# jgsimard/big-dreamer

Hardware: AMD Instinct MI355X
Metric: latent transitions/sec (RSSM + imagination) at batch=50 chunk=50 H=15 (higher is better)
Workload: dtype f32

## Files before the change

### big_dreamer_amd/csrc/bd_device.h

```cpp
#pragma once
#include <hip/hip_runtime.h>
#include <stdint.h>

#include "../../include/bigdreamer_hip.h"

namespace bd {

typedef float floatx4 __attribute__((ext_vector_type(4)));

#ifndef BD_WAVES
#define BD_WAVES 4
#endif
constexpr int kWaves = BD_WAVES;
constexpr int kThreads = kWaves * 64;
constexpr int kFragFloats = 256;

__device__ __forceinline__ floatx4 mfma16(float a, float b, floatx4 c) {
    return __builtin_amdgcn_mfma_f32_16x16x4f32(a, b, c, 0, 0, 0);
}

__host__ __device__ __forceinline__ int cdiv(int a, int b) { return (a + b - 1) / b; }

__device__ __forceinline__ int bd_tid() {
    int t = threadIdx.x;
// ... 313 lines not shown
                return f;
            },
            [&](const LinFrag<RT, NI>& f) {
                if constexpr (kSplit) {
                    if constexpr (TR) {
                        acc[0][0] = mfma16(f.b[0][0], f.a[0][0], acc[0][0]);
                        acc2 = mfma16(f.b[0][1], f.a[0][1], acc2);
                        acc[0][0] = mfma16(f.b[0][2], f.a[0][2], acc[0][0]);
                        acc2 = mfma16(f.b[0][3], f.a[0][3], acc2);
                    } else {
                        acc[0][0] = mfma16(f.a[0][0], f.b[0][0], acc[0][0]);
                        acc2 = mfma16(f.a[0][1], f.b[0][1], acc2);
                        acc[0][0] = mfma16(f.a[0][2], f.b[0][2], acc[0][0]);
                        acc2 = mfma16(f.a[0][3], f.b[0][3], acc2);
                    }
                } else {
#pragma unroll
                    for (int j = 0; j < 4; ++j)
#pragma unroll
                        for (int i = 0; i < NI; ++i)
#pragma unroll
                            for (int rt = 0; rt < RT; ++rt)
                                acc[i][rt] = TR ? mfma16(f.b[i][j], f.a[rt][j], acc[i][rt]) : mfma16(f.a[rt][j], f.b[i][j], acc[i][rt]);
                }
            });
    }
    if constexpr (kSplit) acc[0][0] += acc2;
}

template <int NSEG, int RT, int NI, int D, bool TR = false, class Pre, class Epi>
__device__ __forceinline__ void linear_blocks(const Seg (&seg)[NSEG], const float* __restrict__ bias, int N, int nb0,
                                              Pre&& pre, Epi&& epi, int sb = -1) {
    const int lane = bd_tid() & 63;
    BD_DSTAMP(sb, 0);
    decltype(pre(0, 0)) pf[NI][RT];
#pragma unroll
    for (int i = 0; i < NI; ++i)
#pragma unroll
        for (int rt = 0; rt < RT; ++rt) pf[i][rt] = pre(rt, nb0 + i * kWaves);
    floatx4 acc[NI][RT];
#pragma unroll
    for (int i = 0; i < NI; ++i) {
        floatx4 b4;
        if constexpr (TR) {
            b4 = tall_bias(bias, N, nb0 + i * kWaves, lane);
        } else {
            const int col = (nb0 + i * kWaves) * 16 + (lane & 15);
            const float b = (bias != nullptr && col < N) ? bias[col] : 0.f;
            b4 = floatx4{b, b, b, b};
        }
#pragma unroll
        for (int rt = 0; rt < RT; ++rt) acc[i][rt] = b4;
    }
    BD_DSTAMP(sb, 1);
    linear_sweep<NSEG, RT, NI, D, TR>(seg, nb0, acc);
    BD_DSTAMP(sb, 2);
#pragma unroll
    for (int i = 0; i < NI; ++i)
#pragma unroll
        for (int rt = 0; rt < RT; ++rt) epi(rt, nb0 + i * kWaves, acc[i][rt], pf[i][rt]);
    BD_DSTAMP(sb, 3);
}

constexpr int kSplitPairs = 2;
constexpr int kHeadMaxN = 64;
constexpr int kHeadPlainFloats = 2 * 16 * kHeadMaxN;
constexpr int kSplitPartialFloats = kWaves * kSplitPairs * 2 * kFragFloats;
constexpr int kSplitScratchFloats = kSplitPartialFloats + kHeadPlainFloats;

template <int RT, int NSEG, bool TR = false, class Pre, class Epi>
__device__ __forceinline__ void tile_linear_splitk(const Seg (&seg)[NSEG], const float* __restrict__ bias, int N,
                                                   float* __restrict__ scratch, Pre&& pre, Epi&& epi) {
    const int lane = bd_tid() & 63, wave = bd_wave(bd_tid());
    const int Nb = (N + 15) >> 4;
    const int P = Nb * RT;
    const int my_nb = wave / RT, my_rt = wave - my_nb * RT;
    decltype(pre(0, 0)) pf{};
    floatx4 my_bias = floatx4{0.f, 0.f, 0.f, 0.f};
    if (wave < P) {
        pf = pre(my_rt, my_nb);
        if constexpr (TR) {
            my_bias = tall_bias(bias, N, my_nb, lane);
        } else {
            const int col = my_nb * 16 + (lane & 15);
            const float b = (bias != nullptr && col < N) ? bias[col] : 0.f;
            my_bias = floatx4{b, b, b, b};
        }
    }
    floatx4 acc[kSplitPairs];
#pragma unroll
    for (int p = 0; p < kSplitPairs; ++p) acc[p] = floatx4{0.f, 0.f, 0.f, 0.f};
    constexpr int KW = 2;
#pragma unroll
    for (int s = 0; s < NSEG; ++s) {
        const int Kb = seg[s].Kb;
        const floatx4* __restrict__ X4 = reinterpret_cast<const floatx4*>(seg[s].X) + lane;
        const floatx4* __restrict__ W4 = reinterpret_cast<const floatx4*>(seg[s].W) + lane;
        for (int kb0 = wave; kb0 < Kb; kb0 += kWaves * KW) {
            floatx4 xa[KW][kSplitPairs], wb[KW][kSplitPairs];
#pragma unroll
            for (int i = 0; i < KW; ++i) {
                const int kb = kb0 + i * kWaves;
#pragma unroll
                for (int p = 0; p < kSplitPairs; ++p) {
                    if (kb < Kb && p < P) {
                        const int nb = p / RT, rt = p % RT;
                        xa[i][p] = X4[(rt * Kb + kb) * 64];
                        wb[i][p] = W4[((size_t)nb * Kb + kb) * 64];
                    }
                }
            }
#pragma unroll
            for (int i = 0; i < KW; ++i) {
                const int kb = kb0 + i * kWaves;
#pragma unroll
                for (int p = 0; p < kSplitPairs; ++p) {
                    if (kb < Kb && p < P) {
#pragma unroll
                        for (int j = 0; j < 4; ++j)
                            acc[p] = TR ? mfma16(wb[i][p][j], xa[i][p][j], acc[p]) : mfma16(xa[i][p][j], wb[i][p][j], acc[p]);
                    }
                }
            }
        }
    }
    floatx4* __restrict__ S4 = reinterpret_cast<floatx4*>(scratch);
#pragma unroll
    for (int p = 0; p < kSplitPairs; ++p)
        if (p < P) S4[(wave * kSplitPairs + p) * 64 + lane] = acc[p];
    lds_barrier();
    if (wave < P) {
        floatx4 r = my_bias;
        for (int w = 0; w < kWaves; ++w) r += S4[(w * kSplitPairs + wave) * 64 + lane];
        epi(my_rt, my_nb, r, pf);
    }
}

template <int RT, int NSEG, bool TR = false, class Pre, class Epi>
__device__ __forceinline__ void tile_linear_pre(const Seg (&seg)[NSEG], const float* __restrict__ bias, int N, Pre&& pre,
                                                Epi&& epi, float* __restrict__ scratch = nullptr, int sb = -1) {
    const int wave = bd_wave(bd_tid());
    const int Nb = (N + 15) >> 4;
    if (scratch != nullptr && Nb * RT <= kSplitPairs) {
        tile_linear_splitk<RT, NSEG, TR>(seg, bias, N, scratch, pre, epi);
        return;
    }
#ifndef BD_PIPE_D
#define BD_PIPE_D 2
#endif
    constexpr int D = BD_PIPE_D;
    for (int nb0 = wave; nb0 < Nb; nb0 += 2 * kWaves) {
        if (nb0 + kWaves < Nb) linear_blocks<NSEG, RT, 2, D, TR>(seg, bias, N, nb0, pre, epi, sb);
        else linear_blocks<NSEG, RT, 1, D, TR>(seg, bias, N, nb0, pre, epi, sb);
    }
}

template <int RT, int NSEG, class Epi>
__device__ __forceinline__ void tile_linear_g(const Seg (&seg)[NSEG], const float* __restrict__ bias, int N, Epi&& epi,
                                              float* __restrict__ scratch = nullptr, int sb = -1) {
    tile_linear_pre<RT, NSEG>(seg, bias, N, NoPre{}, [&](int rt, int nb, floatx4 acc, NoPreVal) { epi(rt, nb, acc); },
                              scratch, sb);
}

template <int RT, class Epi>
__device__ __forceinline__ void tile_linear(const float* __restrict__ X, int Kb, const float* __restrict__ Wp,
                                            const float* __restrict__ bias, int N, Epi&& epi,
                                            float* __restrict__ scratch = nullptr) {
    const Seg seg[1] = {{X, Wp, Kb}};
    tile_linear_g<RT, 1>(seg, bias, N, epi, scratch);
}

template <int NSEG, class Epi>
__device__ __forceinline__ void tile_linear_seg(const Seg (&seg)[NSEG], const float* __restrict__ bias, int N,
                                                Epi&& epi, float* __restrict__ scratch = nullptr, int sb = -1) {
    tile_linear_g<1, NSEG>(seg, bias, N, [&](int, int nb, floatx4 acc) { epi(nb, acc); }, scratch, sb);
}
template <int NSEG, class Epi>
__device__ __forceinline__ void tile_linear_seg_tr(const Seg (&seg)[NSEG], const float* __restrict__ bias, int N, Epi&& epi,
                                                   int sb = -1) {
    tile_linear_pre<1, NSEG, true>(seg, bias, N, NoPre{}, [&](int, int nb, floatx4 acc, NoPreVal) { epi(nb, acc); }, nullptr, sb);
}

constexpr int kTallMaxPer = 3;

template <int RT>
struct TallAcc {
    floatx4 main[kTallMaxPer][RT];
    floatx4 left;
};

__host__ __device__ __forceinline__ bool tall_shape_ok(int N, int RT) {
    const int Nb = (N + 15) >> 4, per = Nb / kWaves;
    return per <= kTallMaxPer && (Nb - per * kWaves) * RT <= kWaves;
}

__device__ __forceinline__ bool tall_left_pair(int Nb, int RT, int wave, int& rt, int& nb) {
    const int per = Nb / kWaves, nleft = (Nb - per * kWaves) * RT;
    if (wave >= nleft) return false;
    const int lb = wave / RT;
    rt = wave - lb * RT;
    nb = per * kWaves + lb;
    return true;
}

template <int RT, int NSEG>
__device__ __forceinline__ void tall_sweep(const Seg (&seg)[NSEG], const float* __restrict__ bias, int N, TallAcc<RT>& t) {
    const int lane = bd_tid() & 63, wave = bd_wave(bd_tid());
    const int Nb = (N + 15) >> 4, per = Nb / kWaves;
#pragma unroll
    for (int i = 0; i < kTallMaxPer; ++i) {
        const floatx4 b = i < per ? tall_bias(bias, N, wave + i * kWaves, lane) : floatx4{0.f, 0.f, 0.f, 0.f};
#pragma unroll
        for (int rt = 0; rt < RT; ++rt) t.main[i][rt] = b;
    }
    if (per == 3) linear_sweep<NSEG, RT, 3, 1, true>(seg, wave, t.main);
    else if (per == 2) linear_sweep<NSEG, RT, 2, 1, true>(seg, wave, t.main);
    else if (per == 1) linear_sweep<NSEG, RT, 1, 2, true>(seg, wave, t.main);
    int lrt = 0, lnb = 0;
    if (tall_left_pair(Nb, RT, wave, lrt, lnb)) {
        floatx4 one[1][1] = {{tall_bias(bias, N, lnb, lane)}};
        Seg s1[NSEG];
#pragma unroll
        for (int s = 0; s < NSEG; ++s) s1[s] = Seg{seg[s].X + (size_t)lrt * seg[s].Kb * kFragFloats, seg[s].W, seg[s].Kb};
        linear_sweep<NSEG, 1, 1, 2, true>(s1, lnb, one);
        t.left = one[0][0];
    }
}

template <int RT, class F>
__device__ __forceinline__ void tall_foreach(int N, const TallAcc<RT>& t, F&& f) {
    const int wave = bd_wave(bd_tid());
    const int Nb = (N + 15) >> 4, per = Nb / kWaves;
#pragma unroll
    for (int i = 0; i < kTallMaxPer; ++i)
        if (i < per) {
#pragma unroll
            for (int rt = 0; rt < RT; ++rt) f(rt, wave + i * kWaves, t.main[i][rt]);
        }
    int lrt = 0, lnb = 0;
    if (tall_left_pair(Nb, RT, wave, lrt, lnb)) f(lrt, lnb, t.left);
}

template <int RT, class G>
__device__ __forceinline__ void tall_fill(int N, TallAcc<RT>& t, G&& g) {
    const int wave = bd_wave(bd_tid());
    const int Nb = (N + 15) >> 4, per = Nb / kWaves;
#pragma unroll
    for (int i = 0; i < kTallMaxPer; ++i)
        if (i < per) {
#pragma unroll
            for (int rt = 0; rt < RT; ++rt) t.main[i][rt] = g(rt, wave + i * kWaves);
        }
    int lrt = 0, lnb = 0;
    if (tall_left_pair(Nb, RT, wave, lrt, lnb)) t.left = g(lrt, lnb);
}

template <int RT, class F>
__device__ __forceinline__ void tall_foreach2(int N, const TallAcc<RT>& t, const TallAcc<RT>& u, F&& f) {
    const int wave = bd_wave(bd_tid());
    const int Nb = (N + 15) >> 4, per = Nb / kWaves;
#pragma unroll
    for (int i = 0; i < kTallMaxPer; ++i)
        if (i < per) {
#pragma unroll
            for (int rt = 0; rt < RT; ++rt) f(rt, wave + i * kWaves, t.main[i][rt], u.main[i][rt]);
        }
    int lrt = 0, lnb = 0;
    if (tall_left_pair(Nb, RT, wave, lrt, lnb)) f(lrt, lnb, t.left, u.left);
}

struct Seg2 {
    const float* X;
    const float* W0;
    const float* W1;
    int Kb;
};

struct DualFrag {
    floatx4 a, p, q;
};

template <int NSEG, class Pre, class Epi>
__device__ __forceinline__ void tile_linear_dual_pre(const Seg2 (&seg)[NSEG], const float* __restrict__ bias0,
                                                     const float* __restrict__ bias1, int N, Pre&& pre, Epi&& epi,
                                                     float* __restrict__ scratch = nullptr, int sb = -1) {
    const int lane = bd_tid() & 63, wave = bd_wave(bd_tid());
    const int Nb = (N + 15) >> 4;
    if (scratch != nullptr && Nb <= kSplitPairs) {
        BD_DSTAMP(sb, 0);
        decltype(pre(0)) pf{};
        float mb0 = 0.f, mb1 = 0.f;
        if (wave < Nb) {
            pf = pre(wave);
            const int col = wave * 16 + (lane & 15);
            mb0 = (bias0 != nullptr && col < N) ? bias0[col] : 0.f;
            mb1 = (bias1 != nullptr && col < N) ? bias1[col] : 0.f;
        }
        floatx4 a0[kSplitPairs], a1[kSplitPairs];
#pragma unroll
        for (int p = 0; p < kSplitPairs; ++p) a0[p] = a1[p] = floatx4{0.f, 0.f, 0.f, 0.f};
        constexpr int KW = 2;
#pragma unroll
        for (int s = 0; s < NSEG; ++s) {
            const int Kb = seg[s].Kb;
            const floatx4* __restrict__ X4 = reinterpret_cast<const floatx4*>(seg[s].X) + lane;
            const floatx4* __restrict__ W0 = reinterpret_cast<const floatx4*>(seg[s].W0) + lane;
// ... 359 lines not shown
```

### big_dreamer_amd/csrc/bd_scan.h

```cpp
#pragma once
#include "bd_device.h"

namespace bd {

struct EntConst {
    float mean, sd, inv_var, inv_sd, base0;
};
__device__ __forceinline__ EntConst entropy_const(float mean, float sd) {
    constexpr float kLogSqrt2Pi = 0.91893853320467274f, kLn2 = 0.69314718055994531f;
    return EntConst{mean, sd, 1.f / (sd * sd), 1.f / sd, -logf(sd) - kLogSqrt2Pi - 2.f * kLn2};
}
__device__ __forceinline__ void entropy_sample(const EntConst& c, float e, float& lp, float& dm, float& ds) {
    constexpr float kClamp = 0.99999994f;
    const float u = c.mean + c.sd * e;
    const float y = tanhf(u);
    const float yc = fminf(fmaxf(y, -kClamp), kClamp);
    const float a = 1.f + yc, b = 1.f - yc;
    const float xh = 0.5f * logf(a / b);
    const float diff = xh - c.mean;
    const float t = -2.f * xh;
    const float ex = expf(t);
    const float sp = t > 20.f ? t : log1pf(ex);
    const float sg = t > 20.f ? 1.f : ex / (1.f + ex);
    lp = c.base0 - 0.5f * diff * diff * c.inv_var + 2.f * (xh + sp);
    const float gx = -diff * c.inv_var + 2.f - 4.f * sg;
    const bool pass = (y >= -kClamp) && (y <= kClamp);
    const float J = pass ? (1.f - y * y) / (a * b) : 0.f;
    dm = diff * c.inv_var + gx * J;
    ds = diff * diff * c.inv_var * c.inv_sd - c.inv_sd + gx * J * e;
}


struct HiddenEpi {
    float* dst;
    float* save;
    size_t tn;
    int width, rows, row0, lane;
    __device__ __forceinline__ void operator()(int nb, floatx4 acc) const {
        const int c = lane & 15, q = lane >> 4;
        float* __restrict__ p = dst + acc_frag_off(nb, lane, 0);
        if (row0 + 16 <= rows && nb * 16 + 16 <= width) {
            float v[4];
#pragma unroll
            for (int r = 0; r < 4; ++r) v[r] = elu(acc[r]);
#pragma unroll
            for (int r = 0; r < 4; ++r) p[4 * r] = v[r];
            if (save) {
                float* __restrict__ s = save + tn * width + ((unsigned)(row0 + 4 * q) * (unsigned)width + (unsigned)(nb * 16 + c));
#pragma unroll
                for (int r = 0; r < 4; ++r) st_save(s + (unsigned)r * (unsigned)width, v[r]);
            }
            return;
        }
        const int col = nb * 16 + c;
#pragma unroll
        for (int r = 0; r < 4; ++r) {
            const int grow = row0 + 4 * q + r;
            const bool ok = grow < rows && col < width;
            const float v = ok ? elu(acc[r]) : 0.f;
            p[4 * r] = v;
            if (ok && save) save[(tn + grow) * width + col] = v;
        }
    }
};

struct HiddenEpiTR {
    float* dst;
    float* save;
    size_t tn;
    int width, rows, row0, lane;
    __device__ __forceinline__ void operator()(int nb, floatx4 acc) const {
        const int row = lane & 15, col0 = nb * 16 + 4 * (lane >> 4);
        const bool rok = row0 + row < rows;
        floatx4 v;
#pragma unroll
        for (int r = 0; r < 4; ++r) v[r] = (rok && col0 + r < width) ? elu(acc[r]) : 0.f;
        reinterpret_cast<floatx4*>(dst)[nb * 64 + lane] = v;
        if (save && rok && col0 < width) {
            float* __restrict__ s = save + (tn + row0 + row) * width + col0;
            if (col0 + 4 <= width) {
                __builtin_memcpy(s, &v, 16);
            } else {
#pragma unroll
                for (int r = 0; r < 4; ++r)
                    if (col0 + r < width) s[r] = v[r];
            }
        }
    }
};

struct DpreEpi {
    float* dst;
    float* out;
    size_t tn;
    int width, rows, row0, lane;
    __device__ __forceinline__ void operator()(int, int nb, floatx4 acc, const Pre4& p) const {
        const int c = lane & 15, q = lane >> 4;
        if (row0 + 16 <= rows && nb * 16 + 16 <= width) {
            float v[4];
#pragma unroll
            for (int r = 0; r < 4; ++r) v[r] = acc[r] * elu_grad_from_out(p.v[r]);
            if (out) {
                float* __restrict__ s = out + tn * width + ((unsigned)(row0 + 4 * q) * (unsigned)width + (unsigned)(nb * 16 + c));
#pragma unroll
                for (int r = 0; r < 4; ++r) s[(unsigned)r * (unsigned)width] = v[r];
            }
            if (dst) {
                float* __restrict__ w = dst + acc_frag_off(nb, lane, 0);
#pragma unroll
                for (int r = 0; r < 4; ++r) w[4 * r] = v[r];
            }
            return;
        }
        const int col = nb * 16 + c;
#pragma unroll
        for (int r = 0; r < 4; ++r) {
            const int grow = row0 + 4 * q + r;
            float v = 0.f;
            if (grow < rows && col < width) {
                v = acc[r] * elu_grad_from_out(p.v[r]);
                if (out) out[(tn + grow) * width + col] = v;
            }
            if (dst) dst[acc_frag_off(nb, lane, r)] = v;
        }
    }
};
struct DprePre {
    const float* saved;
    size_t tn;
    int width, rows, row0, lane;
    __device__ __forceinline__ Pre4 operator()(int, int nb) const {
        Pre4 p;
        const int c = lane & 15, q = lane >> 4;
        if (row0 + 16 <= rows && nb * 16 + 16 <= width) {
            const float* __restrict__ s = saved + tn * width + ((unsigned)(row0 + 4 * q) * (unsigned)width + (unsigned)(nb * 16 + c));
#pragma unroll
            for (int r = 0; r < 4; ++r) p.v[r] = s[(unsigned)r * (unsigned)width];
            return p;
        }
        const int col = nb * 16 + c;
#pragma unroll
        for (int r = 0; r < 4; ++r) {
            const int grow = row0 + 4 * q + r;
            p.v[r] = (grow < rows && col < width) ? saved[(tn + grow) * width + col] : 1.f;
        }
        return p;
    }
};

struct PreAct {
    float act[4], th[4], sg[4], dm[4], ds[4], eps[4];
};

}
```

### big_dreamer_amd/csrc/imagine.hip

```cpp
#include "bd_device.h"
#include "bd_host.h"
#include "bd_scan.h"
#include "bd_rng.h"
#include "bd_discrete.h"

namespace bd {

constexpr int kMaxA = 64;

#ifdef BD_STAMPS
__device__ unsigned long long g_stamps[64];
#define BD_STAMP(slot)                                                                      \
    do {                                                                                    \
        if (blockIdx.x == BD_STAMP_WG && threadIdx.x == 0 && t == 3) g_stamps[slot] = __builtin_amdgcn_s_memtime(); \
    } while (0)
#ifndef BD_STAMP_WG
#define BD_STAMP_WG 0
#endif
#else
#define BD_STAMP(slot)
#endif

struct ImgDims {
    int Kb_h, Kb_s, Kb_a, Kb_hd;
// ... 200 lines not shown
                const bool ok = grow < a.N && col < a.Be;
                h_nxt[off] = ok ? hn : 0.f;
                if (ok) {
                    a.feat[(tn + grow) * F + col] = hn;
                    if (a.sv_gates) {
                        float* g = a.sv_gates + (tn + grow) * 4 * a.Be + col;
                        g[0] = rr; g[a.Be] = zz; g[2 * a.Be] = nn; g[3 * a.Be] = NH[r];
                    }
                }
            }
        }, scratch);
        BD_STAMP(9);
        lds_barrier();
        BD_STAMP(10);
        BD_KARGS_FRESH(ap);
        {
            const Seg segs[1] = {{h_nxt, a.w_p1, d.Kb_h}};
            tile_linear_seg_tr<1>(segs, a.b_p1, a.Hd, hidden_epi(bufA, a.sv_p, tn, a.Hd));
        }
        BD_STAMP(11);
        lds_barrier();
        BD_STAMP(12);
        BD_KARGS_FRESH(ap);
        {
            const Seg2 segs[1] = {{bufA, a.w_p2m, a.w_p2s, d.Kb_hd}};
            tile_dual_head_elem<1>(
                segs, a.b_p2, a.b_p2 + a.S, a.S, scratch,
                [&](int row, int col) { return row0 + row < a.N ? a.eps_prior[(tn + row0 + row) * a.S + col] : 0.f; },
                [&](int row, int col, float Mn, float Rw, float eps) {
                    const int grow = row0 + row;
                    float st = 0.f;
                    if (grow < a.N) {
                        const size_t i = (tn + grow) * a.S + col;
                        const float sd = softplusf(Rw) + a.min_std;
                        st = Mn + sd * eps;
                        if (a.prior_mean) a.prior_mean[i] = Mn;
                        a.prior_std[i] = sd;
                        a.feat[(tn + grow) * F + a.Be + col] = st;
                    }
                    sf[frag_idx(row, col)] = st;
                },
                t == 3 ? 8 : -1);
        }
        BD_STAMP(13);
        lds_barrier();
        BD_STAMP(14);
        float* tmp = h_cur; h_cur = h_nxt; h_nxt = tmp;
    }
#undef a
}

constexpr int kEntParts = 16;
template <bool RNG>
__global__ __launch_bounds__(64 * kEntParts) void actor_entropy_kernel(const float* __restrict__ eps, float* __restrict__ stats,
                                                            float* __restrict__ entropy, int Hm, int N, int A, int ns, Rng rng) {
    __shared__ float red[kEntParts][64][3];
    __shared__ float lpj[64];
    const int lane = threadIdx.x & 63, part = threadIdx.x >> 6;
    const int rows_pb = 64 / A;
    const int rl = lane / A, j = lane - rl * A;
    const long row = (long)blockIdx.x * rows_pb + rl;
    const bool valid = rl < rows_pb && row < (long)Hm * N;
    float lp = 0.f, dm = 0.f, ds = 0.f;
    if (valid) {
        const int t = (int)(row / N), n = (int)(row - (long)t * N);
        const float* st = stats + (size_t)row * 4 * A + j;
        const EntConst ec = entropy_const(st[2 * A], st[3 * A]);
        if constexpr (RNG) {
            const int mine = (ns - part + kEntParts - 1) / kEntParts;
            const uint64_t base = (((uint64_t)row * A + j) * kEntParts + part) * (uint64_t)((ns / kEntParts + 4) / 4);
            for (int k0 = 0; k0 < mine; k0 += 4) {
                float e[4];
                rng_normal4(rng, base + (k0 >> 2), e);
#pragma unroll
                for (int q = 0; q < 4; ++q)
                    if (k0 + q < mine) {
                        float l1, d1, d2;
                        entropy_sample(ec, e[q], l1, d1, d2);
                        lp += l1; dm += d1; ds += d2;
                    }
            }
        } else {
            const float* e0 = eps + ((size_t)t * ns * N + n) * A + j;
            for (int k = part; k < ns; k += kEntParts) {
                float l1, d1, d2;
                entropy_sample(ec, e0[(size_t)k * N * A], l1, d1, d2);
                lp += l1; dm += d1; ds += d2;
            }
        }
    }
    red[part][lane][0] = lp; red[part][lane][1] = dm; red[part][lane][2] = ds;
    __syncthreads();
    const float inv_ns = 1.f / (float)ns;
    if (part == 0) {
        float a0 = 0.f, a1 = 0.f, a2 = 0.f;
        for (int w = 0; w < kEntParts; ++w) { a0 += red[w][lane][0]; a1 += red[w][lane][1]; a2 += red[w][lane][2]; }
        lpj[lane] = a0;
        if (valid) {
            float* st = stats + (size_t)row * 4 * A + j;
            st[2 * A] = -a1 * inv_ns;
            st[3 * A] = -a2 * inv_ns;
        }
    }
    __syncthreads();
    if (part == 0 && valid && j == 0) {
        float s = 0.f;
        for (int jj = 0; jj < A; ++jj) s += lpj[lane + jj];
        entropy[row] = -s * inv_ns;
    }
}

__global__ __launch_bounds__(kThreads) void imagine_bwd_kernel(bd_imagine_bwd_args a_) {
    extern __shared__ __attribute__((aligned(16))) float smem[];
    BD_KARGS(bd_imagine_bwd_args, ap);
#define a (*ap)
    const ImgDims d(a.Be, a.S, a.A, a.Hd);
    const int row0 = blockIdx.x * 16;
    const int F = a.Be + a.S, A = a.A;
    const int nh = d.Kb_h * kFragFloats, nhd = d.Kb_hd * kFragFloats, ns = d.Kb_s * kFragFloats,
              na = d.Kb_a * kFragFloats;
    float* dhc = smem;
    float* dR = dhc + nh;
    float* dZ = dR + nh;
    float* dNI = dZ + nh;
    float* dNH = dNI + nh;
    float* dE = dNH + nh;
    float* dP = dE + nh;
    float* bufA = dP + nhd;
    float* bufB = bufA + nhd;
    float* dM = bufB + nhd;
    float* dRaw = dM + ns;
    float* dAm = dRaw + ns;
    float* dAr = dAm + na;
    float* ds_plain = dAr + na;
    float* scratch = ds_plain + 16 * a.S;

    if (a.d_carry_in == nullptr) {
        for (int i = threadIdx.x; i < nh; i += blockDim.x) dhc[i] = 0.f;
        for (int i = threadIdx.x; i < 16 * a.S; i += blockDim.x) ds_plain[i] = 0.f;
    } else {
        for (int i = threadIdx.x; i < 16 * d.Kb_h * 16; i += blockDim.x) {
            const int r = i / (d.Kb_h * 16), k = i - r * (d.Kb_h * 16);
            dhc[frag_idx(r, k)] = (row0 + r < a.N && k < a.Be) ? a.d_carry_in[(size_t)(row0 + r) * F + k] : 0.f;
        }
        for (int i = threadIdx.x; i < 16 * a.S; i += blockDim.x) {
            const int r = i / a.S, k = i - r * a.S;
            ds_plain[i] = (row0 + r < a.N) ? a.d_carry_in[(size_t)(row0 + r) * F + a.Be + k] : 0.f;
        }
    }
    lds_barrier();

    const size_t act_stride = (size_t)a.Hm * a.N * a.Hd;

    for (int t = a.t_end - 1; t >= a.t_begin; --t) {
        const size_t tn = (size_t)t * a.N;
        const int tid = bd_tid();
        const int lane = tid & 63, wave = bd_wave(tid);
        auto dpre_epi = [&](float* dst, float* out, size_t tn_, int width) {
            return DpreEpi{dst, out, tn_, width, a.N, row0, lane};
        };
        auto dpre_pre = [&](const float* saved, size_t tn_, int width) {
            return DprePre{saved, tn_, width, a.N, row0, lane};
        };
        BD_KARGS_FRESH(ap);
        BD_STAMP(20);
        for (int i = tid; i < 16 * d.Kb_s * 16; i += blockDim.x) {
            const int r = i / (d.Kb_s * 16), k = i - r * (d.Kb_s * 16);
            const int grow = row0 + r;
            float dm = 0.f, dr = 0.f;
            if (grow < a.N && k < a.S) {
                const size_t idx = (tn + grow) * a.S + k;
                dm = ds_plain[r * a.S + k] + a.dfeat[(tn + grow) * F + a.Be + k];
                dr = dm * a.eps_prior[idx] * one_minus_exp_neg(a.prior_std[idx] - a.min_std);
            }
            dM[frag_idx(r, k)] = dm;
            dRaw[frag_idx(r, k)] = dr;
        }
        lds_barrier();
        BD_KARGS_FRESH(ap);
        BD_STAMP(21);
        {
            const Seg segs[2] = {{dM, a.wt_p2m, d.Kb_s}, {dRaw, a.wt_p2s, d.Kb_s}};
            tile_linear_pre<1, 2>(segs, nullptr, a.Hd, dpre_pre(a.sv_p, tn, a.Hd), dpre_epi(dP, nullptr, tn, a.Hd));
        }
        lds_barrier();
        BD_KARGS_FRESH(ap);
        BD_STAMP(22);
        {
            const Seg segs3[1] = {{dP, a.wt_p1, d.Kb_hd}};
            tile_linear_pre<1, 1>(
                segs3, nullptr, a.Be,
                [&](int, int nb) {
                    PreGate p;
                    const int col = nb * 16 + (lane & 15);
#pragma unroll
                    for (int r = 0; r < 4; ++r) {
                        const int grow = row0 + 4 * (lane >> 4) + r;
                        const bool ok = grow < a.N && col < a.Be;
                        const float* g = a.sv_gates + (tn + grow) * 4 * a.Be + col;
                        p.r[r] = ok ? g[0] : 0.f;
                        p.z[r] = ok ? g[a.Be] : 0.f;
                        p.n[r] = ok ? g[2 * a.Be] : 0.f;
                        p.hn[r] = ok ? g[3 * a.Be] : 0.f;
                        p.hprev[r] = !ok ? 0.f : (t > 0 ? a.feat[(tn - a.N + grow) * F + col]
                                                        : a.start_feat[(size_t)grow * F + col]);
                        p.dfeat[r] = ok ? a.dfeat[(tn + grow) * F + col] : 0.f;
                    }
                    return p;
                },
                [&](int, int nb, floatx4 acc, const PreGate& p) {
                    const int col = nb * 16 + (lane & 15);
#pragma unroll
                    for (int r = 0; r < 4; ++r) {
                        const int grow = row0 + 4 * (lane >> 4) + r;
                        const int off = acc_frag_off(nb, lane, r);
                        float vr = 0.f, vz = 0.f, vni = 0.f, vnh = 0.f, carry = 0.f;
                        if (grow < a.N && col < a.Be) {
                            const float dh = acc[r] + dhc[off] + p.dfeat[r];
                            const float rr = p.r[r], zz = p.z[r], nn = p.n[r], hn = p.hn[r];
                            const float dn = dh * (1.f - zz);
                            const float dz = dh * (p.hprev[r] - nn);
                            vni = dn * (1.f - nn * nn);
                            vnh = vni * rr;
                            vr = vni * hn * rr * (1.f - rr);
                            vz = dz * zz * (1.f - zz);
                            carry = dh * zz;
                        }
                        dR[off] = vr; dZ[off] = vz; dNI[off] = vni; dNH[off] = vnh;
                        dhc[off] = carry;
                    }
                });
        }
        lds_barrier();
        BD_KARGS_FRESH(ap);
        BD_STAMP(23);
        const GruWT gw{a.wt_ir, a.wt_iz, a.wt_in, a.wt_hr, a.wt_hz, a.wt_hn};
        gru_tile_bwd(
            dR, dZ, dNI, dNH, d.Kb_h, a.Be, gw,
            [&](int nb) {
                Pre4 p;
                const int col = nb * 16 + (lane & 15);
#pragma unroll
                for (int r = 0; r < 4; ++r) {
                    const int grow = row0 + 4 * (lane >> 4) + r;
                    p.v[r] = (grow < a.N && col < a.Be) ? a.sv_x[(tn + grow) * a.Be + col] : 1.f;
                }
                return p;
            },
            [&](int nb, floatx4 DX, floatx4 DH, const Pre4& p) {
                const int col = nb * 16 + (lane & 15);
#pragma unroll
                for (int r = 0; r < 4; ++r) {
                    const int grow = row0 + 4 * (lane >> 4) + r;
                    const int off = acc_frag_off(nb, lane, r);
                    float de = 0.f;
                    if (grow < a.N && col < a.Be) {
                        de = DX[r] * elu_grad_from_out(p.v[r]);
                        dhc[off] += DH[r];
                    }
                    dE[off] = de;
                }
            }, scratch);
        lds_barrier();
        BD_KARGS_FRESH(ap);
        BD_STAMP(24);
        tile_linear<1>(dE, d.Kb_h, a.wt_embed_s, nullptr, a.S, [&](int, int nb, floatx4 acc) {
            const int col = nb * 16 + (lane & 15);
#pragma unroll
            for (int r = 0; r < 4; ++r) {
                const int row = 4 * (lane >> 4) + r;
                if (col < a.S) ds_plain[row * a.S + col] = (row0 + row < a.N) ? acc[r] : 0.f;
            }
        }, scratch);
        lds_barrier();
        if (a.discrete_actions) {
            const Seg segs5[1] = {{dE, a.wt_embed_a, d.Kb_h}};
            tile_linear_pre<1, 1>(segs5, nullptr, A, NoPre{}, [&](int, int nb, floatx4 acc, NoPreVal) {
                const int col = nb * 16 + (lane & 15);
#pragma unroll
                for (int r = 0; r < 4; ++r)
                    if (col < A) dAr[(4 * (lane >> 4) + r) * A + col] = acc[r];
            }, scratch);
            lds_barrier();
            disc_rows_bwd(dAr, a.sv_act_stats, a.dentropy, a.ent_weight, a.d_actor_out, tn, row0, a.N, A, lane, wave);
        } else {
            const Seg segs5[1] = {{dE, a.wt_embed_a, d.Kb_h}};
            tile_linear_pre<1, 1>(
                segs5, nullptr, A,
                [&](int, int nb) {
                    PreAct p;
                    const int col = nb * 16 + (lane & 15);
#pragma unroll
                    for (int r = 0; r < 4; ++r) {
                        const int grow = row0 + 4 * (lane >> 4) + r;
                        const bool ok = grow < a.N && col < A;
                        const size_t i = (tn + grow) * A + col;
                        const float* st = a.sv_act_stats + (tn + grow) * 4 * A + col;
                        p.act[r] = ok ? a.action[i] : 0.f;
                        p.eps[r] = ok ? a.eps_action[i] : 0.f;
                        p.th[r] = ok ? st[0] : 0.f;
                        p.sg[r] = ok ? st[A] : 0.f;
                        p.dm[r] = ok ? st[2 * A] : 0.f;
                        p.ds[r] = ok ? st[3 * A] : 0.f;
                    }
                    return p;
                },
                [&](int, int nb, floatx4 acc, const PreAct& p) {
                    const int col = nb * 16 + (lane & 15);
#pragma unroll
                    for (int r = 0; r < 4; ++r) {
                        const int grow = row0 + 4 * (lane >> 4) + r;
                        float gm = 0.f, gr = 0.f;
                        if (grow < a.N && col < A) {
                            const float dxa = acc[r] * (1.f - p.act[r] * p.act[r]);
                            const float dent = a.ent_weight ? a.dentropy * a.ent_weight[tn + grow] : a.dentropy;
                            const float dmean = dxa + dent * p.dm[r];
                            const float dstd = dxa * p.eps[r] + dent * p.ds[r];
                            gm = dmean * (1.f - p.th[r] * p.th[r]);
                            gr = dstd * p.sg[r];
                            a.d_actor_out[(tn + grow) * 2 * A + col] = gm;
                            a.d_actor_out[(tn + grow) * 2 * A + A + col] = gr;
                        }
                        dAm[acc_frag_off(nb, lane, r)] = gm;
                        dAr[acc_frag_off(nb, lane, r)] = gr;
                    }
                },
                scratch);
        }
        lds_barrier();
        BD_KARGS_FRESH(ap);
        BD_STAMP(25);
        if (a.d_actor_pre != nullptr) {
        {
            const Seg segs[2] = {{dAm, a.wt_a4m, d.Kb_a}, {dAr, a.wt_a4s, d.Kb_a}};
            tile_linear_pre<1, 2>(segs, nullptr, a.Hd, dpre_pre(a.sv_actor + 3 * act_stride, tn, a.Hd),
                                  dpre_epi(bufA, a.d_actor_pre + 3 * act_stride, tn, a.Hd));
        }
        lds_barrier();
        {
            float* src = bufA;
            float* dst = bufB;
            for (int l = 2; l >= 0; --l) {
                const Seg segs[1] = {{src, a.wt_a[l], d.Kb_hd}};
                tile_linear_pre<1, 1>(segs, nullptr, a.Hd, dpre_pre(a.sv_actor + l * act_stride, tn, a.Hd),
                                      dpre_epi(l > 0 ? dst : nullptr, a.d_actor_pre + l * act_stride, tn, a.Hd));
                lds_barrier();
                float* tmp = src; src = dst; dst = tmp;
            }
        }
        }
        BD_STAMP(26);
    }
    BD_KARGS_FRESH(ap);
    if (a.d_carry_out != nullptr) {
        for (int i = threadIdx.x; i < 16 * d.Kb_h * 16; i += blockDim.x) {
            const int r = i / (d.Kb_h * 16), k = i - r * (d.Kb_h * 16);
            if (row0 + r < a.N && k < a.Be) a.d_carry_out[(size_t)(row0 + r) * F + k] = dhc[frag_idx(r, k)];
        }
        for (int i = threadIdx.x; i < 16 * a.S; i += blockDim.x) {
            const int r = i / a.S, k = i - r * a.S;
            if (row0 + r < a.N) a.d_carry_out[(size_t)(row0 + r) * F + a.Be + k] = ds_plain[i];
        }
    }
#undef a
}

}

extern "C" {
using namespace bd;

#ifdef BD_STAMPS
int bd_debug_stamps(unsigned long long* out64) {
    return hipMemcpyFromSymbol(out64, HIP_SYMBOL(g_stamps), sizeof(unsigned long long) * 64) == hipSuccess ? 0 : -1;
}
int bd_debug_dstamps(unsigned long long* out64) {
    return hipMemcpyFromSymbol(out64, HIP_SYMBOL(g_dstamps), sizeof(unsigned long long) * 64) == hipSuccess ? 0 : -1;
}
#endif

static int imagine_forward_scan(const bd_imagine_fwd_args* a, void* stream) {
    BD_REQUIRE(a && a->N > 0 && a->Hm > 0 && a->Be > 0 && a->S > 0 && a->A > 0 && a->A <= kMaxA && a->Hd > 0 &&
                   a->n_samples > 0, "bd_imagine_forward: bad dims");
    BD_REQUIRE(a->S <= kHeadMaxN && a->A <= kHeadMaxN, "bd_imagine_forward: state / action width above %d", kHeadMaxN);
    BD_REQUIRE(a->w_embed_s && a->w_embed_a && a->b_embed && a->w_ir && a->w_iz && a->w_in && a->w_hr && a->w_hz &&
                   a->w_hn && a->b_ih && a->b_hh && a->w_p1 && a->b_p1 && a->w_p2m && a->w_p2s && a->b_p2,
               "bd_imagine_forward: missing world-model weights");
    BD_REQUIRE(a->w_a0h && a->w_a0s && a->w_a[0] && a->w_a[1] && a->w_a[2] && a->b_a[0] && a->b_a[1] && a->b_a[2] &&
                   a->b_a[3] && a->w_a4m && (a->w_a4s || a->discrete_actions) && a->b_a4,
               "bd_imagine_forward: missing actor weights");
    BD_REQUIRE(!a->discrete_actions || a->sv_act_us == nullptr,
               "bd_imagine_forward: sv_act_us is for the tanh-Normal actor only (discrete_actions = 1 saves norm in sv_act_stats)");
    BD_REQUIRE(a->start_feat && a->eps_action && a->eps_prior && (a->eps_entropy || a->sv_act_stats || a->discrete_actions),
               "bd_imagine_forward: missing inputs (eps_entropy may be NULL only with sv_act_stats: the entropy estimate is then "
               "the caller's bd_actor_entropy / bd_actor_entropy_rng launch)");
    BD_REQUIRE(a->feat && a->prior_std && a->entropy && a->action, "bd_imagine_forward: missing outputs");
    const ImgDims d(a->Be, a->S, a->A, a->Hd);
    const size_t lds = ((size_t)(3 * d.Kb_h + 2 * d.Kb_hd + d.Kb_s + d.Kb_a) * kFragFloats +
                        (size_t)(3 * 16 + kWaves * 16 * 3) * a->A + kSplitScratchFloats) * sizeof(float);
    BD_REQUIRE(lds <= (size_t)kMaxLds, "bd_imagine_forward: needs %zu B of LDS", lds);
    if (lds > 64 * 1024 && allow_big_lds(imagine_fwd_kernel)) return -1;
    hipLaunchKernelGGL(imagine_fwd_kernel, dim3(cdiv(a->N, 16)), dim3(kThreads), lds, (hipStream_t)stream, *a);
    BD_CHECK_LAUNCH("bd_imagine_forward");
    return 0;
}

int bd_actor_entropy(const float* eps_entropy, float* act_stats, float* entropy, int Hm, int N, int A, int n_samples,
                     void* stream) {
    BD_REQUIRE(eps_entropy && act_stats && entropy && Hm > 0 && N > 0 && A > 0 && A <= kMaxA && n_samples > 0,
               "bd_actor_entropy: bad arguments");
    const int rows_pb = 64 / A;
    hipLaunchKernelGGL(actor_entropy_kernel<false>, dim3(cdiv(Hm * N, rows_pb)), dim3(64 * kEntParts), 0, (hipStream_t)stream,
                       eps_entropy, act_stats, entropy, Hm, N, A, n_samples, Rng{0, 0, 0, 0});
    BD_CHECK_LAUNCH("bd_actor_entropy");
    return 0;
}

int bd_actor_entropy_rng(unsigned long long seed, unsigned long long step, unsigned stream_id, float* act_stats, float* entropy,
                         int Hm, int N, int A, int n_samples, void* stream) {
    BD_REQUIRE(act_stats && entropy && Hm > 0 && N > 0 && A > 0 && A <= kMaxA && n_samples > 0, "bd_actor_entropy_rng: bad arguments");
    const int rows_pb = 64 / A;
    hipLaunchKernelGGL(actor_entropy_kernel<true>, dim3(cdiv(Hm * N, rows_pb)), dim3(64 * kEntParts), 0, (hipStream_t)stream,
                       nullptr, act_stats, entropy, Hm, N, A, n_samples,
                       Rng{(uint32_t)seed, (uint32_t)(seed >> 32), stream_id, (uint32_t)step});
    BD_CHECK_LAUNCH("bd_actor_entropy_rng");
    return 0;
}

int bd_imagine_forward_scan(const bd_imagine_fwd_args* a, void* stream) { return imagine_forward_scan(a, stream); }

int bd_imagine_forward(const bd_imagine_fwd_args* a, void* stream) {
    if (int rc = imagine_forward_scan(a, stream)) return rc;
    if (a->sv_act_stats != nullptr && a->eps_entropy != nullptr && !a->discrete_actions)
        return bd_actor_entropy(a->eps_entropy, a->sv_act_stats, a->entropy, a->Hm, a->N, a->A, a->n_samples, stream);
    return 0;
}

int bd_imagine_backward(const bd_imagine_bwd_args* a, void* stream) {
    BD_REQUIRE(a && a->N > 0 && a->Hm > 0 && a->Be > 0 && a->S > 0 && a->A > 0 && a->A <= kMaxA && a->Hd > 0,
               "bd_imagine_backward: bad dims");
    BD_REQUIRE(a->wt_embed_s && a->wt_embed_a && a->wt_ir && a->wt_iz && a->wt_in && a->wt_hr && a->wt_hz && a->wt_hn &&
                   a->wt_p1 && a->wt_p2m && a->wt_p2s && a->wt_a[0] && a->wt_a[1] && a->wt_a[2] &&
                   (a->discrete_actions || (a->wt_a4m && a->wt_a4s)),
               "bd_imagine_backward: missing weights");
    BD_REQUIRE(!a->discrete_actions || a->d_actor_pre == nullptr,
               "bd_imagine_backward: the Categorical actor's hidden layers run as the caller's chain (d_actor_pre = NULL)");
    BD_REQUIRE(a->start_feat && a->feat && a->prior_std && a->action && (a->eps_action || a->discrete_actions) &&
                   a->eps_prior && a->sv_actor &&
                   a->sv_act_stats && a->sv_x && a->sv_gates && a->sv_p && a->dfeat,
               "bd_imagine_backward: missing forward tensors");
    BD_REQUIRE(a->d_actor_out, "bd_imagine_backward: missing outputs");
    bd_imagine_bwd_args w = *a;
    if (w.t_begin == 0 && w.t_end == 0) w.t_end = w.Hm;
    BD_REQUIRE(0 <= w.t_begin && w.t_begin < w.t_end && w.t_end <= w.Hm,
               "bd_imagine_backward: bad window [t_begin = %d, t_end = %d) of Hm = %d steps", a->t_begin, a->t_end, a->Hm);
    BD_REQUIRE((w.d_carry_in != nullptr) == (w.t_end < w.Hm),
               "bd_imagine_backward: d_carry_in is needed exactly when t_end < Hm (t_end = %d, Hm = %d)", w.t_end, w.Hm);
    BD_REQUIRE((w.d_carry_out != nullptr) == (w.t_begin > 0),
               "bd_imagine_backward: d_carry_out is needed exactly when t_begin > 0 (t_begin = %d)", w.t_begin);
    const ImgDims d(a->Be, a->S, a->A, a->Hd);
    const size_t lds = ((size_t)(6 * d.Kb_h + 3 * d.Kb_hd + 2 * d.Kb_s + 2 * d.Kb_a) * kFragFloats + 16 * a->S +
                        kSplitPartialFloats) * sizeof(float);
    BD_REQUIRE(lds <= (size_t)kMaxLds, "bd_imagine_backward: needs %zu B of LDS", lds);
    if (lds > 64 * 1024 && allow_big_lds(imagine_bwd_kernel)) return -1;
    hipLaunchKernelGGL(imagine_bwd_kernel, dim3(cdiv(a->N, 16)), dim3(kThreads), lds, (hipStream_t)stream, w);
    BD_CHECK_LAUNCH("bd_imagine_backward");
    return 0;
}

}
```

Baseline: 13.63 million.

## Prefetch backward-scan epilogue operands ahead of barriers and next timestep

In the backward imagination scan, the operands each wave's first linear blocks need (saved hidden activations, gate values, sample eps/std/dfeat) are now loaded into registers before the LDS barrier. The loads are clamped so they need no guards. The per-thread sample operands for the next timestep are also prefetched a step early. A new tile_linear_ahead helper takes these preloaded values for the first block pair, so global-load latency overlaps the barrier and the previous stage. This costs extra registers and adds a debug probe macro that can pin operand reads to a single timestep.

```diff
diff --git a/big_dreamer_amd/csrc/bd_device.h b/big_dreamer_amd/csrc/bd_device.h
--- a/big_dreamer_amd/csrc/bd_device.h
+++ b/big_dreamer_amd/csrc/bd_device.h
@@ -489,6 +489,23 @@
     for (int nb0 = wave; nb0 < Nb; nb0 += 2 * kWaves) {
         if (nb0 + kWaves < Nb) linear_blocks<NSEG, RT, 2, D, TR>(seg, bias, N, nb0, pre, epi, sb);
         else linear_blocks<NSEG, RT, 1, D, TR>(seg, bias, N, nb0, pre, epi, sb);
+    }
+}
+
+template <int NSEG, class P, class Pre, class Epi>
+__device__ __forceinline__ void tile_linear_ahead(const Seg (&seg)[NSEG], const float* __restrict__ bias, int N,
+                                                  const P (&ahead)[2], Pre&& pre, Epi&& epi) {
+    const int wave = bd_wave(bd_tid());
+    const int Nb = (N + 15) >> 4;
+    constexpr int D = BD_PIPE_D;
+    if (wave < Nb) {
+        auto first = [&](int, int nb) { return nb == wave ? ahead[0] : ahead[1]; };
+        if (wave + kWaves < Nb) linear_blocks<NSEG, 1, 2, D>(seg, bias, N, wave, first, epi);
+        else linear_blocks<NSEG, 1, 1, D>(seg, bias, N, wave, first, epi);
+    }
+    for (int nb0 = wave + 2 * kWaves; nb0 < Nb; nb0 += 2 * kWaves) {
+        if (nb0 + kWaves < Nb) linear_blocks<NSEG, 1, 2, D>(seg, bias, N, nb0, pre, epi);
+        else linear_blocks<NSEG, 1, 1, D>(seg, bias, N, nb0, pre, epi);
     }
 }
 
diff --git a/big_dreamer_amd/csrc/bd_scan.h b/big_dreamer_amd/csrc/bd_scan.h
--- a/big_dreamer_amd/csrc/bd_scan.h
+++ b/big_dreamer_amd/csrc/bd_scan.h
@@ -151,5 +151,7 @@
 struct PreAct {
     float act[4], th[4], sg[4], dm[4], ds[4], eps[4];
 };
-
+struct PreSample {
+    float dfeat, eps, std;
+};
 }
diff --git a/big_dreamer_amd/csrc/imagine.hip b/big_dreamer_amd/csrc/imagine.hip
--- a/big_dreamer_amd/csrc/imagine.hip
+++ b/big_dreamer_amd/csrc/imagine.hip
@@ -376,8 +376,28 @@
 
     const size_t act_stride = (size_t)a.Hm * a.N * a.Hd;
 
+    auto sample_pre = [&](size_t tn_, int i) {
+        const int r = i / (d.Kb_s * 16), k = i - r * (d.Kb_s * 16);
+        const int grow = row0 + r;
+        const bool ok = i < 16 * d.Kb_s * 16 && grow < a.N && k < a.S;
+        const size_t idx = (tn_ + grow) * a.S + k;
+        PreSample p;
+        p.dfeat = ok ? a.dfeat[(tn_ + grow) * F + a.Be + k] : 0.f;
+        p.eps = ok ? a.eps_prior[idx] : 0.f;
+        p.std = ok ? a.prior_std[idx] : 0.f;
+        return p;
+    };
+#ifdef BD_STAGE_PROBE
+#define BD_OPERAND_STEP(t_) (a.t_end - 1)
+#else
+#define BD_OPERAND_STEP(t_) (t_)
+#endif
+    PreSample sample_ahead = sample_pre((size_t)BD_OPERAND_STEP(a.t_end - 1) * a.N, bd_tid());
+    const bool offsets32 = (size_t)a.N * (size_t)(4 * a.Be + F + a.Hd) < ((size_t)1 << 31);
+
     for (int t = a.t_end - 1; t >= a.t_begin; --t) {
         const size_t tn = (size_t)t * a.N;
+        const size_t tnl = (size_t)BD_OPERAND_STEP(t) * a.N;
         const int tid = bd_tid();
         const int lane = tid & 63, wave = bd_wave(tid);
         auto dpre_epi = [&](float* dst, float* out, size_t tn_, int width) {
@@ -386,6 +406,31 @@
         auto dpre_pre = [&](const float* saved, size_t tn_, int width) {
             return DprePre{saved, tn_, width, a.N, row0, lane};
         };
+        auto saved_pre = [&](const float* saved, int width, int nb) {
+            if (offsets32 && row0 + 16 <= a.N && nb * 16 + 16 <= width) return dpre_pre(saved, tnl, width)(0, nb);
+            Pre4 p;
+            const float* __restrict__ s = saved + tnl * width + min(nb * 16 + (lane & 15), width - 1);
+#pragma unroll
+            for (int r = 0; r < 4; ++r) p.v[r] = s[(size_t)min(row0 + 4 * (lane >> 4) + r, a.N - 1) * width];
+            return p;
+        };
+        auto gate_pre = [&](int nb) {
+            PreGate p;
+            const int col = min(nb * 16 + (lane & 15), a.Be - 1);
+            const float* __restrict__ h0 = t > 0 ? a.feat + (tnl - a.N) * F : a.start_feat;
+#pragma unroll
+            for (int r = 0; r < 4; ++r) {
+                const size_t grow = (size_t)min(row0 + 4 * (lane >> 4) + r, a.N - 1);
+                const float* __restrict__ g = a.sv_gates + (tnl + grow) * 4 * a.Be + col;
+                p.r[r] = g[0];
+                p.z[r] = g[a.Be];
+                p.n[r] = g[2 * a.Be];
+                p.hn[r] = g[3 * a.Be];
+                p.hprev[r] = h0[grow * F + col];
+                p.dfeat[r] = a.dfeat[(tnl + grow) * F + col];
+            }
+            return p;
+        };
         BD_KARGS_FRESH(ap);
         BD_STAMP(20);
         for (int i = tid; i < 16 * d.Kb_s * 16; i += blockDim.x) {
@@ -393,45 +438,37 @@
             const int grow = row0 + r;
             float dm = 0.f, dr = 0.f;
             if (grow < a.N && k < a.S) {
-                const size_t idx = (tn + grow) * a.S + k;
-                dm = ds_plain[r * a.S + k] + a.dfeat[(tn + grow) * F + a.Be + k];
-                dr = dm * a.eps_prior[idx] * one_minus_exp_neg(a.prior_std[idx] - a.min_std);
+                const PreSample p = i == tid ? sample_ahead : sample_pre(tnl, i);
+                dm = ds_plain[r * a.S + k] + p.dfeat;
+                dr = dm * p.eps * one_minus_exp_neg(p.std - a.min_std);
             }
             dM[frag_idx(r, k)] = dm;
             dRaw[frag_idx(r, k)] = dr;
         }
+        auto hidden_pre = [&](int, int nb) { return saved_pre(a.sv_p, a.Hd, nb); };
+        Pre4 hidden_ahead[2];
+        PreGate gate_ahead[2];
+#pragma unroll
+        for (int i = 0; i < 2; ++i) {
+            const int nb = wave + i * kWaves;
+            hidden_ahead[i] = nb * 16 < a.Hd ? hidden_pre(0, nb) : Pre4{};
+            gate_ahead[i] = nb * 16 < a.Be ? gate_pre(nb) : PreGate{};
+        }
+        if (t > a.t_begin) sample_ahead = sample_pre((size_t)BD_OPERAND_STEP(t - 1) * a.N, tid);
         lds_barrier();
         BD_KARGS_FRESH(ap);
         BD_STAMP(21);
         {
             const Seg segs[2] = {{dM, a.wt_p2m, d.Kb_s}, {dRaw, a.wt_p2s, d.Kb_s}};
-            tile_linear_pre<1, 2>(segs, nullptr, a.Hd, dpre_pre(a.sv_p, tn, a.Hd), dpre_epi(dP, nullptr, tn, a.Hd));
+            tile_linear_ahead(segs, nullptr, a.Hd, hidden_ahead, hidden_pre, dpre_epi(dP, nullptr, tn, a.Hd));
         }
         lds_barrier();
         BD_KARGS_FRESH(ap);
         BD_STAMP(22);
         {
             const Seg segs3[1] = {{dP, a.wt_p1, d.Kb_hd}};
-            tile_linear_pre<1, 1>(
-                segs3, nullptr, a.Be,
-                [&](int, int nb) {
-                    PreGate p;
-                    const int col = nb * 16 + (lane & 15);
-#pragma unroll
-                    for (int r = 0; r < 4; ++r) {
-                        const int grow = row0 + 4 * (lane >> 4) + r;
-                        const bool ok = grow < a.N && col < a.Be;
-                        const float* g = a.sv_gates + (tn + grow) * 4 * a.Be + col;
-                        p.r[r] = ok ? g[0] : 0.f;
-                        p.z[r] = ok ? g[a.Be] : 0.f;
-                        p.n[r] = ok ? g[2 * a.Be] : 0.f;
-                        p.hn[r] = ok ? g[3 * a.Be] : 0.f;
-                        p.hprev[r] = !ok ? 0.f : (t > 0 ? a.feat[(tn - a.N + grow) * F + col]
-                                                        : a.start_feat[(size_t)grow * F + col]);
-                        p.dfeat[r] = ok ? a.dfeat[(tn + grow) * F + col] : 0.f;
-                    }
-                    return p;
-                },
+            tile_linear_ahead(
+                segs3, nullptr, a.Be, gate_ahead, [&](int, int nb) { return gate_pre(nb); },
                 [&](int, int nb, floatx4 acc, const PreGate& p) {
                     const int col = nb * 16 + (lane & 15);
 #pragma unroll
@@ -467,7 +504,7 @@
 #pragma unroll
                 for (int r = 0; r < 4; ++r) {
                     const int grow = row0 + 4 * (lane >> 4) + r;
-                    p.v[r] = (grow < a.N && col < a.Be) ? a.sv_x[(tn + grow) * a.Be + col] : 1.f;
+                    p.v[r] = (grow < a.N && col < a.Be) ? a.sv_x[(tnl + grow) * a.Be + col] : 1.f;
                 }
                 return p;
             },
@@ -518,8 +555,8 @@
                     for (int r = 0; r < 4; ++r) {
                         const int grow = row0 + 4 * (lane >> 4) + r;
                         const bool ok = grow < a.N && col < A;
-                        const size_t i = (tn + grow) * A + col;
-                        const float* st = a.sv_act_stats + (tn + grow) * 4 * A + col;
+                        const size_t i = (tnl + grow) * A + col;
+                        const float* st = a.sv_act_stats + (tnl + grow) * 4 * A + col;
                         p.act[r] = ok ? a.action[i] : 0.f;
                         p.eps[r] = ok ? a.eps_action[i] : 0.f;
                         p.th[r] = ok ? st[0] : 0.f;
@@ -586,6 +623,7 @@
             if (row0 + r < a.N) a.d_carry_out[(size_t)(row0 + r) * F + a.Be + k] = ds_plain[i];
         }
     }
+#undef BD_OPERAND_STEP
 #undef a
 }
 
```

After: 13.65 million (median of 6 runs). No clear change (+0.2%).
